# ZhiHuangHn/vtkCloudPoint

Hardware: AMD Instinct MI355X
Metric: Mpoints/s DBSCAN+label @10M pts (higher is better)
Workload: dtype f64; 1 GPU; C4: 10000000-pt cloud (half uniform background, 200 Gaussian blobs), one monolithic DBImproved.dbscan, metric L1_2D, eps 0.1, minPts 10; mode=single, points_total=10000000, points_per_gpu=10000000, clusters=27380, resident_in_hbm=True

## Files before the change

### include/vcp.h

```cpp
#ifndef VCP_H
#define VCP_H
#include <stdint.h>

#ifdef __cplusplus
extern "C" {
#endif

#define VCP_VERSION_MAJOR 0
#define VCP_VERSION_MINOR 1

typedef struct vcp_ctx vcp_ctx;

enum vcp_metric { VCP_L1_2D = 0, VCP_L2_2D = 1, VCP_L2_3D = 2, VCP_SIGNED_SUM_2D = 3 };

enum vcp_icp_stop { VCP_STOP_SSE_DELTA = 0, VCP_STOP_RMSE = 1 };

enum vcp_status {
  VCP_OK = 0,
  VCP_ERR_ARG = -1,
  VCP_ERR_EMPTY = -2,
  VCP_ERR_DEGENERATE = -3,
  VCP_ERR_INDEX = -4,
  VCP_ERR_TOO_LARGE = -5,
  VCP_ERR_NO_DEVICE = -6,
// ... 1 lines not shown
  VCP_ERR_UNSUPPORTED = -8,
  VCP_ERR_NOMEM = -9
};

int vcp_create(int device_id, vcp_ctx** out);
void vcp_destroy(vcp_ctx* ctx);
const char* vcp_last_error(const vcp_ctx* ctx);
int vcp_version(void);
int vcp_set_stream(vcp_ctx* ctx, void* hip_stream);
int vcp_dev_alloc(vcp_ctx* ctx, uint64_t bytes, void** dptr);
int vcp_dev_free(vcp_ctx* ctx, void* dptr);
int vcp_h2d(vcp_ctx* ctx, void* dst_dev, const void* src_host, uint64_t bytes);
int vcp_d2h(vcp_ctx* ctx, void* dst_host, const void* src_dev, uint64_t bytes);

int vcp_release_workspace(vcp_ctx* ctx);

int vcp_selftest_scan_dev(vcp_ctx* ctx, const uint32_t* d_in, uint32_t* d_out, int64_t n, int op, uint32_t* total);

int vcp_selftest_horn(const double sums[16], int64_t nd, double V[16], int use_v, double R1[9], double T1[3]);

int vcp_timing_enable(vcp_ctx* ctx, int on);
int vcp_timing_count(vcp_ctx* ctx);
int vcp_timing_get(vcp_ctx* ctx, int i, const char** name, float* ms);

int vcp_dbscan(vcp_ctx* ctx, const double* coords, int64_t n, int dim, int metric, double eps,
               int min_pts, int32_t cf_in, const uint8_t* in_mask, const uint8_t* in_classed,
               int32_t* labels, uint8_t* is_core, uint8_t* is_classed, int32_t* cf_out,
               int64_t* dist_evals);
int vcp_dbscan_dev(vcp_ctx* ctx, const double* d_coords, int64_t n, int dim, int metric, double eps,
                   int min_pts, int32_t cf_in, const uint8_t* d_in_classed, int32_t* d_labels,
// ... 166 lines not shown
```

### vtkcloudpoint_amd/_native.py

```python
import ctypes as C
import os

import numpy as np

_HERE = os.path.dirname(os.path.abspath(__file__))
LIB_PATH = os.path.join(_HERE, "libvcp.so")

L1_2D, L2_2D, L2_3D, SIGNED_SUM_2D = 0, 1, 2, 3
STOP_SSE_DELTA, STOP_RMSE = 0, 1

STATUS = {
    0: "VCP_OK", -1: "VCP_ERR_ARG", -2: "VCP_ERR_EMPTY", -3: "VCP_ERR_DEGENERATE", -4: "VCP_ERR_INDEX",
    -5: "VCP_ERR_TOO_LARGE", -6: "VCP_ERR_NO_DEVICE", -7: "VCP_ERR_HIP", -8: "VCP_ERR_UNSUPPORTED",
    -9: "VCP_ERR_NOMEM",
}

SYMBOLS = [
    "vcp_create", "vcp_destroy", "vcp_last_error", "vcp_version", "vcp_set_stream", "vcp_dev_alloc",
    "vcp_dev_free", "vcp_h2d", "vcp_d2h", "vcp_timing_enable", "vcp_timing_count", "vcp_timing_get",
    "vcp_dbscan", "vcp_dbscan_dev", "vcp_dbscan_blocks", "vcp_blocks_begin", "vcp_blocks_begin_dev",
    "vcp_blocks_share", "vcp_blocks_cluster_dev", "vcp_blocks_finish_dev", "vcp_centroids", "vcp_centroids_dev",
    "vcp_merge_centroids", "vcp_refresh_by_dictionary", "vcp_icp", "vcp_icp_dev", "vcp_icp_sums",
    "vcp_match", "vcp_mcc", "vcp_assign_truths", "vcp_icp_vtklike", "vcp_import_convert",
    "vcp_slab_begin", "vcp_slab_comps", "vcp_slab_finish", "vcp_release_workspace", "vcp_selftest_scan_dev",
    "vcp_centroids_weighted", "vcp_dbscan_blocks_keyed", "vcp_blocks_begin_keyed", "vcp_blocks_begin_keyed_dev",
    "vcp_selftest_horn", "vcp_create_multi", "vcp_destroy_multi", "vcp_multi_last_error", "vcp_multi_count",
    "vcp_multi_ctx", "vcp_dbscan_blocks_multi", "vcp_blocks_share_plan", "vcp_blocks_plan_dev", "vcp_blocks_plan_cuts",
    "vcp_blocks_build_dev", "vcp_blocks_finish_local_dev", "vcp_blocks_finish_zero_dev", "vcp_blocks_finish_zcoords_dev",
    "vcp_blocks_finish_pairs_dev", "vcp_scatter_pairs_dev", "vcp_kdist", "vcp_kdist_dev", "vcp_icp_multistart",
    "vcp_cluster_shapes", "vcp_cluster_shapes_dev", "vcp_cluster_filter", "vcp_cluster_filter_dev",
    "vcp_icp_sums_gated", "vcp_icp_gated", "vcp_match_unique", "vcp_match_unique_dev",
    "vcp_register_pairs", "vcp_register_pairs_dev", "vcp_selftest_register_pose",
]


class VcpError(RuntimeError):
    def __init__(self, code, msg):
        super().__init__("%s (%d): %s" % (STATUS.get(code, "?"), code, msg))
        self.code = code


_lib = None


def lib():
    global _lib
    if _lib is None:
        if not os.path.exists(LIB_PATH):
# ... 653 lines not shown
```

### vtkcloudpoint_amd/csrc/dbscan.hip

```cpp
#include <string.h>

#include <cmath>
#include <cstdlib>
#include <cstring>
#include <limits>
#include <vector>

#include "bounds.hpp"
#include "dbscan_engine.hpp"
#include "grid_common.hpp"

using namespace vcpg;

namespace {

#ifndef VCP_UNR2
#define VCP_UNR2 4
#endif
#ifndef VCP_UNR3
#define VCP_UNR3 2
#endif
#ifndef VCP_UNRW
#define VCP_UNRW 4
#endif
// ... 118 lines not shown
  uint32_t perblk;
  uint32_t nblk;
};

__device__ __forceinline__ uint32_t wl_fetch(const WorkList& w) {
  const uint32_t total = w.scan[w.nblk] - w.scan[0];
  const uint32_t x = blockIdx.x & 7u, i = blockIdx.x >> 3;
  const uint32_t c = (i / w.perblk) * 8u + x;
  const uint32_t lo = (uint32_t)(((uint64_t)total * c) / (8u * LCHUNK));
  const uint32_t hi = (uint32_t)(((uint64_t)total * (c + 1u)) / (8u * LCHUNK));
  const uint32_t t = lo + (i % w.perblk) * TPB + threadIdx.x;
  if (t >= hi) return NONE;
  return w.list[t];
}

__device__ __forceinline__ void wl_count(bool isE, bool isB, uint32_t blk, uint32_t* __restrict__ cntE,
                                         uint32_t* __restrict__ cntB) {
  __shared__ unsigned wc[2][TPB / 64];
  const unsigned long long mE = __ballot(isE), mB = __ballot(isB);
  if ((threadIdx.x & 63) == 0) {
    wc[0][threadIdx.x >> 6] = (unsigned)__popcll(mE);
    wc[1][threadIdx.x >> 6] = (unsigned)__popcll(mB);
  }
  __syncthreads();
  if (threadIdx.x == 0) {
    unsigned a = 0, b = 0;
    for (int k = 0; k < TPB / 64; k++) {
      a += wc[0][k];
      b += wc[1][k];
    }
// ... 46 lines not shown
  int NB;
  int core_cap;
};

__device__ __forceinline__ void wave_prefix_small(uint32_t v, uint32_t& pre, uint32_t& sum) {
  pre = 0;
  sum = 0;
#pragma unroll
  for (int b = 0; b < 4; b++) {
    const unsigned long long m = __ballot((v >> b) & 1u);
    pre += __builtin_amdgcn_mbcnt_hi((uint32_t)(m >> 32), __builtin_amdgcn_mbcnt_lo((uint32_t)m, 0u)) << b;
    sum += (uint32_t)__popcll(m) << b;
  }
}

__device__ __forceinline__ const uint32_t* nbr_list(const NbrOut& no, uint32_t p) {
  return no.nbr + (size_t)(p / TPB) * (size_t)(no.NB * TPB) + no.off[p];
}

__device__ __forceinline__ void nbr_flush(const NbrOut& no, const uint32_t* lnb, uint32_t* lout, int nrec, int64_t blk,
                                          int64_t p, bool live) {
  if (no.NB == 0) return;
  __shared__ uint32_t wtot[TPB / 64];
  const int lane = threadIdx.x & 63, w = threadIdx.x >> 6;
  uint32_t pre, wsum;
  wave_prefix_small((uint32_t)nrec, pre, wsum);
  if (lane == 0) wtot[w] = wsum;
  __syncthreads();
  uint32_t total = 0;
  for (int k = 0; k < TPB / 64; k++) {
    if (k < w) pre += wtot[k];
    total += wtot[k];
// ... 406 lines not shown
        const uint32_t jj = min(j0 + u, e - 1);
        cand[u] = (j0 + u < e) && (flags[jj] & F_EXPAND);
        if (GROUPED) cand[u] = cand[u] && sgroup[jj] == myg;
        load_pt32<GD>(sorted32, jj, rr[u]);
      }
#pragma unroll
      for (int u = 0; u < UNR; u++)
        if (first == me && cand[u] && within_scr<GD, METRIC>(qf, rr[u], sc, xs, me, j0 + u, thr)) first = j0 + u;
      if (first != me) return false;
    }
    return true;
  });
  if (first != me) parent[me] = first;
}

__global__ __launch_bounds__(TPB) void k_union_init_list(const uint8_t* __restrict__ flags, uint32_t* __restrict__ parent,
                                                        NbrOut no, WorkList wlE) {
  const uint32_t p = wl_fetch(wlE);
  if (p == NONE) return;
  const int nrec = flags[p] >> 4;
  const uint32_t* li = nbr_list(no, p);
  for (int k = 0; k < nrec; k++) {
    const uint32_t j = li[k];
    if (j < p && (flags[j] & F_EXPAND)) {
      parent[p] = j;
      return;
    }
  }
}

template <int JOIN>
__global__ __launch_bounds__(TPB) void k_flatten0(uint32_t* __restrict__ parent, WorkList wlE,
                                                 const uint8_t* __restrict__ flags, NbrOut no) {
  const uint32_t p = wl_fetch(wlE);
  if (p == NONE) return;
  uint32_t r = (uint32_t)p, x = ld_parent_cached(parent, r);
  if (x == r || JOIN == 2) {
    if (!JOIN) return;
    uint32_t rp = JOIN == 2 ? uf_root(parent, p) : p;
    const int nrec = flags[p] >> 4;
    const uint32_t* li = nbr_list(no, p);
    uint32_t s0 = NONE, s1 = NONE, s2 = NONE;
    for (int k = 0; k < nrec; k++) {
      const uint32_t j = li[k];
      if (!(flags[j] & F_EXPAND)) continue;
      const uint32_t y = ld_parent_cached(parent, j);
      if (y == rp || y == s0 || y == s1 || y == s2) continue;
      const uint32_t ry = uf_root(parent, y);
      const uint32_t rm = uf_root(parent, rp);
      s2 = s1;
      s1 = s0;
      s0 = rp;
      rp = (ry != rm) ? uf_link(parent, rm, ry) : rm;
      if (y != rp) s1 = y;
    }
    return;
  }
  while (x != r) {
    r = x;
    x = ld_parent_cached(parent, r);
  }
  __hip_atomic_store(&parent[p], r, __ATOMIC_RELAXED, __HIP_MEMORY_SCOPE_WAVEFRONT);
}

constexpr uint32_t CHUNK_MIXED = 0xFFFFFFFEu;
constexpr int DENSE_PER_CELL = 16;
__global__ __launch_bounds__(TPB) void k_chunkroot(const uint32_t* __restrict__ parent, CellTab ct,
                                                  uint32_t* __restrict__ chunkroot) {
  const uint32_t nin = *ct.nin;
  const int64_t p = (int64_t)blockIdx.x * TPB + threadIdx.x;
  const uint32_t x = p < nin ? parent[p] : NONE;
  const unsigned long long have = __ballot(x != NONE);
  uint32_t out = NONE;
  if (have) {
    const uint32_t r = (uint32_t)__shfl((int)x, __ffsll((long long)have) - 1, 64);
    out = __ballot(x != NONE && x != r) ? CHUNK_MIXED : r;
  }
// ... 90 lines not shown
        } else if (q1 == NONE) {
          q1 = x;
        } else {
          VCP_FLUSH();
          q0 = x;
        }
      }
    }
  }
  VCP_FLUSH();
  if (rp != me) __hip_atomic_store(&parent[me], rp, __ATOMIC_RELAXED, __HIP_MEMORY_SCOPE_AGENT);
}
#undef VCP_FLUSH
#undef VCP_JOIN

template <bool FILTER>
__global__ __launch_bounds__(TPB) void k_flatten(uint32_t* __restrict__ parent, const uint32_t* __restrict__ sord,
                                                uint32_t* __restrict__ minord, WorkList wlE) {
  const uint32_t p = wl_fetch(wlE);
  uint32_t r = NONE, v = NONE;
  if (p != NONE) {
    r = (uint32_t)p;
    uint32_t x = parent[r];
    while (x != r) {
      r = x;
      x = parent[r];
    }
    parent[p] = r;
    v = sord[p];
  }
  unsigned long long todo = __ballot(r != NONE);
  const int lane = threadIdx.x & 63;
  while (todo) {
    int leader = __ffsll((long long)todo) - 1;
    uint32_t lr = __shfl(r, leader, 64);
    bool mine = (r == lr);
    uint32_t m = mine ? v : NONE;
#pragma unroll
    for (int d = 32; d > 0; d >>= 1) m = min(m, (uint32_t)__shfl_xor((int)m, d, 64));
    if (lane == leader &&
        (!FILTER || m < __hip_atomic_load(&minord[lr], __ATOMIC_RELAXED, __HIP_MEMORY_SCOPE_AGENT)))
      atomicMin(&minord[lr], m);
    todo &= ~__ballot(mine);
  }
}

__device__ __forceinline__ uint32_t seed_rank(const uint32_t* __restrict__ bits, const uint32_t* __restrict__ pref,
                                              uint32_t m) {
  const uint32_t w = m >> 5;
  return pref[w] + (uint32_t)__popc(bits[w] & ((1u << (m & 31u)) - 1u));
}
__global__ __launch_bounds__(TPB) void k_seed_popc(const uint32_t* __restrict__ bits, uint32_t nw, uint32_t* __restrict__ cnt) {
  uint32_t w = blockIdx.x * TPB + threadIdx.x;
  if (w < nw) cnt[w] = (uint32_t)__popc(bits[w]);
}

__global__ __launch_bounds__(TPB) void k_seedflag(const uint32_t* __restrict__ parent, const uint32_t* __restrict__ minord,
                                                 uint32_t* __restrict__ seedflag, WorkList wlE) {
  const uint32_t p = wl_fetch(wlE);
  if (p == NONE) return;
  if (parent[p] == p) {
    const uint32_t m = minord[p];
    atomicOr(&seedflag[m >> 5], 1u << (m & 31u));
  }
}

__global__ __launch_bounds__(TPB) void k_rootk(const uint32_t* __restrict__ parent, const uint32_t* __restrict__ minord,
                                              const uint32_t* __restrict__ seedbits, const uint32_t* __restrict__ seedpref,
                                              uint32_t* __restrict__ rootk, uint32_t* __restrict__ clseed, WorkList wlE) {
  const uint32_t p = wl_fetch(wlE);
  if (p == NONE) return;
  if (parent[p] == p) {
    uint32_t k = seed_rank(seedbits, seedpref, minord[p]);
    rootk[p] = k;
    clseed[k] = minord[p];
  }
}

__device__ __forceinline__ void twice_add(unsigned twice, unsigned long long* __restrict__ counters) {
  __shared__ unsigned tw[TPB / 64];
  const unsigned long long m2 = __ballot(twice);
  if ((threadIdx.x & 63) == 0) tw[threadIdx.x >> 6] = (unsigned)__popcll(m2);
  __syncthreads();
  if (threadIdx.x == 0) {
    unsigned t = 0;
    for (int k = 0; k < TPB / 64; k++) t += tw[k];
    if (t) atomicAdd(&counters[CNT_TWICE + (blockIdx.x & (CNT_SPREAD - 1))], (unsigned long long)t);
  }
}

template <int GD, int METRIC, bool GROUPED>
__global__ __launch_bounds__(TPB) void k_border(ExactSrc xs, GridP g, double thr,
                                               CellTab ct,
                                               const int32_t* __restrict__ sgroup, const uint8_t* __restrict__ flags,
                                               const uint32_t* __restrict__ parent, const uint32_t* __restrict__ sord,
                                               const uint32_t* __restrict__ rootk, const uint32_t* __restrict__ clseed,
                                               uint32_t* __restrict__ labk, unsigned long long* __restrict__ counters,
// ... 31 lines not shown
          }
        }
        return true;
      });
      out = mx;
      if (mx != 0 && !(fl & F_CLASSED) && sord[p] - own_lo < own_span && sord[p] < clseed[mnk]) {
        twice = 1;
        if (GROUPED) atomicAdd(&group_twice[myg], 1u);
      }
    }
    labk[p] = (out << 2) | ((fl & F_CORE) ? 1u : 0u) | ((fl & F_CLASSED) ? 2u : 0u);
  }
  if (!GROUPED) twice_add(twice, counters);
}

template <bool GROUPED>
__global__ __launch_bounds__(TPB) void k_border_list(const int32_t* __restrict__ sgroup, const uint8_t* __restrict__ flags,
                                                    const uint32_t* __restrict__ sord, const uint32_t* __restrict__ rootk,
                                                    const uint32_t* __restrict__ clseed, uint32_t* __restrict__ labk,
                                                    unsigned long long* __restrict__ counters,
                                                    uint32_t* __restrict__ group_twice, NbrOut no, WorkList wlB) {
  const uint32_t p = wl_fetch(wlB);
  unsigned twice = 0;
  if (p != NONE) {
    const uint8_t fl = flags[p];
    const int nrec = fl >> 4;
    uint32_t mx = 0, mnk = NONE;
    const uint32_t* li = nbr_list(no, p);
    for (int k = 0; k < nrec; k++) {
      const uint32_t x = rootk[li[k]];
      if (x == NONE) continue;
      mx = max(mx, x + 1u);
      mnk = min(mnk, x);
    }
    if (mx != 0 && sord[p] < clseed[mnk]) twice = 1;
    labk[p] = (mx << 2) | ((fl & F_CORE) ? 1u : 0u) | ((fl & F_CLASSED) ? 2u : 0u);
  }
  if (GROUPED) {
    const int32_t g = twice ? sgroup[p] : -1;
    unsigned long long todo = __ballot(twice != 0);
    const int lane = threadIdx.x & 63;
    while (todo) {
      const int leader = __ffsll((long long)todo) - 1;
      const int32_t gl = __shfl(g, leader, 64);
      const unsigned long long same = __ballot(twice && g == gl);
      if (lane == leader) atomicAdd(&group_twice[gl], (uint32_t)__popcll(same));
      todo &= ~same;
    }
  } else {
    twice_add(twice, counters);
  }
}

__global__ __launch_bounds__(TPB) void k_labk_rest(const uint8_t* __restrict__ flags, const uint32_t* __restrict__ parent,
                                                  uint32_t* rootk, uint32_t* __restrict__ labk,
                                                  CellTab ct) {
  const uint32_t nin = *ct.nin;
  int64_t p = (int64_t)blockIdx.x * TPB + threadIdx.x;
  if (p >= nin) return;
  const uint8_t fl = flags[p];
  uint32_t k = NONE;
  if (fl & F_EXPAND) {
    const uint32_t r = parent[p];
    k = rootk[r];
    if (r != (uint32_t)p) rootk[p] = k;
// ... 244 lines not shown
  if (lo_ok && lo >= 0.0 && std::isfinite(lo)) {
    float l = (float)lo;
    if ((double)l > lo) l = std::nextafterf(l, -INFINITY);
    sc.lo = l;
  } else if (lo_ok && std::isinf(thr) && thr > 0) {
    sc.lo = 3.4028234663852886e38f;
  }
  return sc;
}

unsigned list_perblk(int64_t n) {
  const int64_t band = (n + 8 * LCHUNK - 1) / (8 * LCHUNK) + 1;
  return vcp_blocks(band, TPB);
}

struct Switches {
  int64_t cells_per_point;
  bool screen_off, lists_off, core_global;
  int core_cap, join_all;
};
const Switches& switches() {
  static const Switches sw = [] {
    Switches s;
    const char* e = getenv("VCP_CELL_BUDGET");
    const long v = e ? atol(e) : 32;
    s.cells_per_point = (int64_t)(v < 1 ? 1 : v > 4096 ? 4096 : v);
    s.screen_off = getenv("VCP_NO_SCREEN") != nullptr;
    s.lists_off = getenv("VCP_NO_LISTS") != nullptr;
    s.core_global = getenv("VCP_CORE_GLOBAL") != nullptr;
    s.core_cap = getenv("VCP_CORE_CAP") ? atoi(getenv("VCP_CORE_CAP")) : -1;
    s.join_all = getenv("VCP_JOIN_ALL") ? atoi(getenv("VCP_JOIN_ALL")) : -1;
    return s;
  }();
  return sw;
}

struct EnginePinned {
  double bounds[8];
  uint32_t unclassed;
  uint32_t n_comp;
  unsigned long long counters[CNT_WORDS];
};
static_assert(sizeof(EnginePinned) <= 1024, "the engine's region of vcp_ctx::pinned");
EnginePinned* engine_pinned(vcp_ctx* ctx) { return reinterpret_cast<EnginePinned*>(ctx->pinned); }

struct Call {
// ... 339 lines not shown
  }
  if (!tiled)
    VCP_LAUNCH(ctx, (k_core<GD, METRIC, GROUPED>), dim3(nb), dim3(TPB), 2 * lds_nb, st, c.xs, c.g, c.thr, c.min_pts, ws.ct,
                    ws.sgroup, ws.flags, ws.parent, ws.minord, ws.blkE, ws.blkB, no, ws.sorted32, c.sc, c.flags_set);
  VCP_TRY(vcp_exclusive_scan_u32(ctx, ws.blkE, ws.blkE, 2 * ((int64_t)nb + 2), nullptr));
  VCP_LAUNCH(ctx, k_wl_fill, dim3(nb), dim3(TPB), 0, st, ws.flags, ws.ct, ws.blkE, ws.blkB, ws.wlE.list, ws.wlB.list,
                  ws.seedflag, ws.nw, ws.counters, c.d_group_twice, (uint32_t)(GROUPED ? c.G : 0));
  return VCP_OK;
}

template <int GD, int METRIC, bool GROUPED>
int stage_union(vcp_ctx* ctx, const Call& c, const Workspace& ws, const Switches& sw) {
  hipStream_t st = ctx->stream;
  const int64_t n = c.n;
  const unsigned nb = c.nb, nbl = ws.nbl;
  const GridP& g = c.g;
  const NbrOut& no = c.no;
  vcp_phase(ctx, "union");
  const bool pre = GD == 2 || no.NB > 0;
  if (no.NB > 0) {
    VCP_LAUNCH(ctx, k_union_init_list, dim3(nbl), dim3(TPB), 0, st, ws.flags, ws.parent, no, ws.wlE);
    const bool all = sw.join_all >= 0 ? sw.join_all != 0 : (uint64_t)n >= (uint64_t)g.ncells;
    if (all) VCP_LAUNCH(ctx, k_flatten0<2>, dim3(nbl), dim3(TPB), 0, st, ws.parent, ws.wlE, ws.flags, no);
    else VCP_LAUNCH(ctx, k_flatten0<1>, dim3(nbl), dim3(TPB), 0, st, ws.parent, ws.wlE, ws.flags, no);
    VCP_LAUNCH(ctx, k_flatten0<0>, dim3(nbl), dim3(TPB), 0, st, ws.parent, ws.wlE, ws.flags, no);
  } else if (GD == 2) {
    VCP_LAUNCH(ctx, (k_union_init<GD, METRIC, GROUPED>), dim3(nbl), dim3(TPB), 0, st, c.xs, g, c.thr, ws.ct, ws.sgroup,
                    ws.flags, ws.parent, ws.wlE, ws.sorted32, c.sc);
    VCP_LAUNCH(ctx, k_flatten0<0>, dim3(nbl), dim3(TPB), 0, st, ws.parent, ws.wlE, ws.flags, no);
  }
  const bool dense = pre && (uint64_t)n > (uint64_t)DENSE_PER_CELL * g.ncells;
  if (dense) {
    VCP_TRY(vcp_ensure(ctx, ctx->b_aux0, ((size_t)nb * (TPB / 64) + 2) * 4));
    uint32_t* chunkroot = ctx->b_aux0.as<uint32_t>();
    VCP_LAUNCH(ctx, k_chunkroot, dim3(nb), dim3(TPB), 0, st, ws.parent, ws.ct, chunkroot);
    VCP_LAUNCH(ctx, (k_union<GD, METRIC, GROUPED, true, true>), dim3(nbl), dim3(TPB), 0, st, c.xs, g, c.thr, ws.ct,
                    ws.sgroup, ws.parent, ws.wlE, ws.sorted32, c.sc, chunkroot);
  } else if (pre)
    VCP_LAUNCH(ctx, (k_union<GD, METRIC, GROUPED, true>), dim3(nbl), dim3(TPB), 0, st, c.xs, g, c.thr, ws.ct, ws.sgroup,
                    ws.parent, ws.wlE, ws.sorted32, c.sc);
  else
    VCP_LAUNCH(ctx, (k_union<GD, METRIC, GROUPED, false>), dim3(nbl), dim3(TPB), 0, st, c.xs, g, c.thr, ws.ct, ws.sgroup,
                    ws.parent, ws.wlE, ws.sorted32, c.sc);
  return VCP_OK;
// ... 17 lines not shown
  ss.valid = true;
  ss.gd = c.gd;
  ss.metric = c.metric;
  ss.n = c.n;
  ss.n_comp = hn[0];
  ss.g = c.g;
  ss.thr = c.thr;
  ss.sc = c.sc;
  ss.xs = c.xs;
  ss.nb = nb;
  if (c.cf_out) *c.cf_out = (int32_t)hn[0];
  return VCP_OK;
}

template <bool GROUPED>
int stage_flatten_number(vcp_ctx* ctx, const Call& c, const Workspace& ws) {
  hipStream_t st = ctx->stream;
  const unsigned nbl = ws.nbl;
  vcp_phase(ctx, "flatten_number");
  if ((uint64_t)c.n >= (uint64_t)c.g.ncells)
    VCP_LAUNCH(ctx, k_flatten<true>, dim3(nbl), dim3(TPB), 0, st, ws.parent, ws.sord, ws.minord, ws.wlE);
  else
    VCP_LAUNCH(ctx, k_flatten<false>, dim3(nbl), dim3(TPB), 0, st, ws.parent, ws.sord, ws.minord, ws.wlE);
  if (!GROUPED && c.slab) return stage_slab_handoff(ctx, c, ws);
  VCP_LAUNCH(ctx, k_seedflag, dim3(nbl), dim3(TPB), 0, st, ws.parent, ws.minord, ws.seedflag, ws.wlE);
  VCP_LAUNCH(ctx, k_seed_popc, dim3(vcp_blocks(ws.nw, TPB)), dim3(TPB), 0, st, ws.seedflag, ws.nw, ws.seedpref);
  VCP_TRY(vcp_exclusive_scan_u32(ctx, ws.seedpref, ws.seedpref, ws.nw, ws.d_total));
  VCP_LAUNCH(ctx, k_rootk, dim3(nbl), dim3(TPB), 0, st, ws.parent, ws.minord, ws.seedflag, ws.seedpref, ws.rootk, ws.clseed,
                  ws.wlE);
  return VCP_OK;
}

template <int GD, int METRIC, bool GROUPED>
int stage_border(vcp_ctx* ctx, const Call& c, const Workspace& ws) {
  hipStream_t st = ctx->stream;
  vcp_phase(ctx, "border");
  VCP_LAUNCH(ctx, k_labk_rest, dim3(c.nb), dim3(TPB), 0, st, ws.flags, ws.parent, ws.rootk, ws.labk, ws.ct);
  if (c.no.NB > 0)
    VCP_LAUNCH(ctx, k_border_list<GROUPED>, dim3(ws.nbl), dim3(TPB), 0, st, ws.sgroup, ws.flags, ws.sord, ws.rootk,
                    ws.clseed, ws.labk, ws.counters, c.d_group_twice, c.no, ws.wlB);
  else
    VCP_LAUNCH(ctx, (k_border<GD, METRIC, GROUPED>), dim3(ws.nbl), dim3(TPB), 0, st, c.xs, c.g, c.thr, ws.ct, ws.sgroup,
                    ws.flags, ws.parent, ws.sord, ws.rootk, ws.clseed, ws.labk, ws.counters, c.d_group_twice, ws.wlB, 0u,
                    NONE, ws.sorted32, c.sc);
  return VCP_OK;
}

template <int GD, bool GROUPED>
int stage_output(vcp_ctx* ctx, const Call& c, const Workspace& ws) {
  hipStream_t st = ctx->stream;
  const int64_t n = c.n;
  const unsigned nb = c.nb;
  const DbscanExt* ext = c.ext;
  if (c.part_out) {
    GridOutputArgs oa;
    oa.n = n;
    oa.sord = ws.sord;
    oa.labk = ws.labk;
    oa.have_in_classed = c.d_in_classed != nullptr;
// ... 29 lines not shown
  c.thr = (METRIC == VCP_L1_2D) ? c.eps : l2_threshold(c.eps);
  if (!GROUPED && c.all_finite && !c.slab && box_measure<GD, METRIC>(c.h) <= c.thr) return run_all_pairs(ctx, c);

  double Emax = 0.0;
  VCP_TRY(grid_geometry(ctx, c, sw, Emax));
  c.sc = screen_bounds(METRIC, GD, METRIC == VCP_L1_2D ? c.thr * c.g.scale : c.thr * c.g.scale * c.g.scale, Emax * c.g.scale);
  if (sw.screen_off) c.sc = Screen{-1.0f, INFINITY};

  VCP_TRY(ws_reserve(ctx, c.n, c.nb, GD, GROUPED, c.g.ncells));
  const Workspace ws = ws_carve(ctx, c.n, c.nb, GROUPED, c.g.ncells);
  c.flags_set = c.d_in_classed != nullptr;
  c.part_out = !GROUPED && !c.d_ord && !c.slab && c.n <= ((int64_t)1 << 27);
  VCP_TRY(stage_grid_build(ctx, c, ws));
  VCP_TRY((stage_core<GD, METRIC, GROUPED>(ctx, c, ws, sw)));
  VCP_TRY((stage_union<GD, METRIC, GROUPED>(ctx, c, ws, sw)));
  VCP_TRY(stage_flatten_number<GROUPED>(ctx, c, ws));
  if (!GROUPED && c.slab) return VCP_OK;
  VCP_TRY((stage_border<GD, METRIC, GROUPED>(ctx, c, ws)));
  VCP_TRY((stage_output<GD, GROUPED>(ctx, c, ws)));

  Totals t;
  VCP_TRY(read_totals(ctx, ws, t));
  const unsigned long long unclassed = c.d_in_classed ? t.unclassed : (unsigned long long)c.n;
  if (c.cf_out) *c.cf_out = c.cf_in + (int32_t)t.K;
  if (c.dist_evals)
    *c.dist_evals = GROUPED ? (int64_t)t.group_evals : (int64_t)(unclassed + t.twice + t.K - t.slot0) * c.n;
  return VCP_OK;
}

template <int GD, int METRIC>
int run_slab_finish(vcp_ctx* ctx, const SlabState& ss, const uint32_t* d_map_rep, const uint32_t* d_map_k,
                    const int32_t* d_tab_gid, uint32_t own_lo, uint32_t own_span, int32_t* d_labels,
                    uint8_t* d_is_classed, int64_t* twice) {
// ... 85 lines not shown
  Call c{d_coords, n, stride, metric, eps, min_pts, cf_in, d_in_classed, d_labels, d_is_core, d_is_classed, cf_out,
         dist_evals, ext};
  call_derive(c);
  if (!(eps >= 0.0)) {
    if (grouped) return vcp_fail(ctx, VCP_ERR_ARG, "grouped DBSCAN needs eps >= 0");
    return run_degenerate(ctx, c);
  }
  if (grouped) return run_dbscan<2, VCP_L1_2D, true>(ctx, c);
  if (metric == VCP_L1_2D) return run_dbscan<2, VCP_L1_2D, false>(ctx, c);
  if (metric == VCP_L2_2D) return run_dbscan<2, VCP_L2_2D, false>(ctx, c);
  return run_dbscan<3, VCP_L2_3D, false>(ctx, c);
}

extern "C" {

void vcp_slab_state_free(vcp_ctx* ctx) {
  delete ctx->slab;
  ctx->slab = nullptr;
}

int vcp_slab_begin(vcp_ctx* ctx, const double* d_coords, int64_t n, int dim, int metric, double eps, int min_pts,
                   const uint8_t* d_noexpand, const uint32_t* d_ord, uint32_t* d_rep, uint8_t* d_is_core,
                   int64_t* n_comp) {
  if (!ctx) return VCP_ERR_ARG;
  if (n <= 0) return vcp_fail(ctx, VCP_ERR_ARG, "vcp_slab_begin needs n > 0");
  if (!d_ord || !d_rep || !n_comp) return vcp_fail(ctx, VCP_ERR_ARG, "null buffer");
  if (!(eps >= 0.0) || std::isinf(eps)) return vcp_fail(ctx, VCP_ERR_ARG, "staged DBSCAN needs a finite eps >= 0");
  DbscanExt ext;
  ext.d_ord = d_ord;
  ext.slab = true;
// ... 126 lines not shown
```

Baseline: 7019 Mpoints/s.

## Process multiple worklist entries per thread with batched neighbor-list loads

```diff
diff --git a/include/vcp.h b/include/vcp.h
--- a/include/vcp.h
+++ b/include/vcp.h
@@ -39,6 +39,8 @@
 int vcp_d2h(vcp_ctx* ctx, void* dst_host, const void* src_dev, uint64_t bytes);
 
 int vcp_release_workspace(vcp_ctx* ctx);
+
+int vcp_worklist_entries(void);
 
 int vcp_selftest_scan_dev(vcp_ctx* ctx, const uint32_t* d_in, uint32_t* d_out, int64_t n, int op, uint32_t* total);
 
diff --git a/vtkcloudpoint_amd/_native.py b/vtkcloudpoint_amd/_native.py
--- a/vtkcloudpoint_amd/_native.py
+++ b/vtkcloudpoint_amd/_native.py
@@ -30,8 +30,12 @@
     "vcp_blocks_finish_pairs_dev", "vcp_scatter_pairs_dev", "vcp_kdist", "vcp_kdist_dev", "vcp_icp_multistart",
     "vcp_cluster_shapes", "vcp_cluster_shapes_dev", "vcp_cluster_filter", "vcp_cluster_filter_dev",
     "vcp_icp_sums_gated", "vcp_icp_gated", "vcp_match_unique", "vcp_match_unique_dev",
-    "vcp_register_pairs", "vcp_register_pairs_dev", "vcp_selftest_register_pose",
+    "vcp_register_pairs", "vcp_register_pairs_dev", "vcp_selftest_register_pose", "vcp_worklist_entries",
 ]
+
+
+def worklist_entries():
+    return int(lib().vcp_worklist_entries())
 
 
 class VcpError(RuntimeError):
diff --git a/vtkcloudpoint_amd/csrc/dbscan.hip b/vtkcloudpoint_amd/csrc/dbscan.hip
--- a/vtkcloudpoint_amd/csrc/dbscan.hip
+++ b/vtkcloudpoint_amd/csrc/dbscan.hip
@@ -4,6 +4,7 @@
 #include <cstdlib>
 #include <cstring>
 #include <limits>
+#include <type_traits>
 #include <vector>
 
 #include "bounds.hpp"
@@ -156,6 +157,35 @@
   return w.list[t];
 }
 
+constexpr int WL_EMAX = 4;
+__host__ __device__ constexpr uint32_t wl_perblk(uint32_t perblk, int E) {
+  return (perblk + (uint32_t)E - 1u) / (uint32_t)E;
+}
+template <int E>
+__device__ __forceinline__ void wl_fetch_n(const WorkList& w, uint32_t (&p)[E]) {
+  static_assert(E >= 1 && E <= WL_EMAX, "entries per thread");
+  const uint32_t total = w.scan[w.nblk] - w.scan[0];
+  const uint32_t per = wl_perblk(w.perblk, E);
+  const uint32_t x = blockIdx.x & 7u, i = blockIdx.x >> 3;
+  const uint32_t c = (i / per) * 8u + x;
+  const uint32_t lo = (uint32_t)(((uint64_t)total * c) / (8u * LCHUNK));
+  const uint32_t hi = (uint32_t)(((uint64_t)total * (c + 1u)) / (8u * LCHUNK));
+  const uint32_t t0 = lo + (i % per) * (uint32_t)(E * TPB) + threadIdx.x;
+#pragma unroll
+  for (int e = 0; e < E; e++) {
+    const uint32_t t = t0 + (uint32_t)(e * TPB);
+    const uint32_t v = w.list[t < hi ? t : 0u];
+    p[e] = t < hi ? v : NONE;
+  }
+}
+__device__ __forceinline__ uint32_t wl_safe(uint32_t p) { return p != NONE ? p : 0u; }
+__device__ __forceinline__ void loaded_here(uint32_t v) { asm volatile("" ::"v"(v)); }
+constexpr int LBATCH = 4;
+__device__ __forceinline__ uint32_t list_word(const uint32_t* li, int nrec, int k, const uint32_t* idle) {
+  const uint32_t* src = nrec > 0 ? li + min(k, nrec - 1) : idle;
+  return *src;
+}
+
 __device__ __forceinline__ void wl_count(bool isE, bool isB, uint32_t blk, uint32_t* __restrict__ cntE,
                                          uint32_t* __restrict__ cntB) {
   __shared__ unsigned wc[2][TPB / 64];
@@ -232,8 +262,8 @@
   }
 }
 
-__device__ __forceinline__ const uint32_t* nbr_list(const NbrOut& no, uint32_t p) {
-  return no.nbr + (size_t)(p / TPB) * (size_t)(no.NB * TPB) + no.off[p];
+__device__ __forceinline__ const uint32_t* nbr_list(const NbrOut& no, uint32_t p, uint32_t of) {
+  return no.nbr + (size_t)(p / TPB) * (size_t)(no.NB * TPB) + of;
 }
 
 __device__ __forceinline__ void nbr_flush(const NbrOut& no, const uint32_t* lnb, uint32_t* lout, int nrec, int64_t blk,
@@ -670,53 +700,137 @@
   if (first != me) parent[me] = first;
 }
 
+template <int E>
 __global__ __launch_bounds__(TPB) void k_union_init_list(const uint8_t* __restrict__ flags, uint32_t* __restrict__ parent,
                                                         NbrOut no, WorkList wlE) {
-  const uint32_t p = wl_fetch(wlE);
-  if (p == NONE) return;
-  const int nrec = flags[p] >> 4;
-  const uint32_t* li = nbr_list(no, p);
-  for (int k = 0; k < nrec; k++) {
-    const uint32_t j = li[k];
-    if (j < p && (flags[j] & F_EXPAND)) {
-      parent[p] = j;
-      return;
-    }
-  }
-}
-
-template <int JOIN>
-__global__ __launch_bounds__(TPB) void k_flatten0(uint32_t* __restrict__ parent, WorkList wlE,
-                                                 const uint8_t* __restrict__ flags, NbrOut no) {
-  const uint32_t p = wl_fetch(wlE);
-  if (p == NONE) return;
-  uint32_t r = (uint32_t)p, x = ld_parent_cached(parent, r);
-  if (x == r || JOIN == 2) {
-    if (!JOIN) return;
-    uint32_t rp = JOIN == 2 ? uf_root(parent, p) : p;
-    const int nrec = flags[p] >> 4;
-    const uint32_t* li = nbr_list(no, p);
-    uint32_t s0 = NONE, s1 = NONE, s2 = NONE;
-    for (int k = 0; k < nrec; k++) {
-      const uint32_t j = li[k];
-      if (!(flags[j] & F_EXPAND)) continue;
-      const uint32_t y = ld_parent_cached(parent, j);
-      if (y == rp || y == s0 || y == s1 || y == s2) continue;
-      const uint32_t ry = uf_root(parent, y);
+  constexpr int LB = E * LBATCH > 8 ? 8 / E : LBATCH;
+  uint32_t p[E];
+  wl_fetch_n<E>(wlE, p);
+  uint8_t fl[E];
+  uint32_t of[E];
+#pragma unroll
+  for (int e = 0; e < E; e++) {
+    fl[e] = flags[wl_safe(p[e])];
+    of[e] = no.off[wl_safe(p[e])];
+  }
+#pragma unroll
+  for (int e = 0; e < E; e++) loaded_here(of[e]);
+  int nrec[E];
+  const uint32_t* li[E];
+  uint32_t first[E];
+#pragma unroll
+  for (int e = 0; e < E; e++) {
+    nrec[e] = p[e] != NONE ? fl[e] >> 4 : 0;
+    li[e] = nbr_list(no, wl_safe(p[e]), of[e]);
+    first[e] = NONE;
+  }
+  for (int k0 = 0;; k0 += LB) {
+    bool more = false;
+#pragma unroll
+    for (int e = 0; e < E; e++) more = more || (first[e] == NONE && k0 < nrec[e]);
+    if (!more) break;
+    uint32_t j[E][LB];
+    uint8_t fj[E][LB];
+#pragma unroll
+    for (int e = 0; e < E; e++)
+#pragma unroll
+      for (int u = 0; u < LB; u++) j[e][u] = list_word(li[e], nrec[e], k0 + u, wlE.list);
+#pragma unroll
+    for (int e = 0; e < E; e++)
+#pragma unroll
+      for (int u = 0; u < LB; u++) {
+        const bool ok = k0 + u < nrec[e] && j[e][u] < p[e];
+        fj[e][u] = flags[ok ? j[e][u] : wl_safe(p[e])];
+        if (!ok) fj[e][u] = 0;
+      }
+#pragma unroll
+    for (int e = 0; e < E; e++)
+#pragma unroll
+      for (int u = 0; u < LB; u++)
+        if (first[e] == NONE && (fj[e][u] & F_EXPAND)) first[e] = j[e][u];
+  }
+#pragma unroll
+  for (int e = 0; e < E; e++)
+    if (first[e] != NONE) parent[p[e]] = first[e];
+}
+
+__device__ __forceinline__ void join_along_list(uint32_t* __restrict__ parent, const uint8_t* __restrict__ flags,
+                                                const NbrOut& no, uint32_t p, uint32_t rp) {
+  const uint8_t fl = flags[p];
+  const uint32_t of = no.off[p];
+  loaded_here(of);
+  const int nrec = fl >> 4;
+  const uint32_t* li = nbr_list(no, p, of);
+  uint32_t s0 = NONE, s1 = NONE, s2 = NONE;
+  for (int k0 = 0; k0 < nrec; k0 += LBATCH) {
+    uint32_t j[LBATCH], y[LBATCH];
+    uint8_t fj[LBATCH];
+#pragma unroll
+    for (int u = 0; u < LBATCH; u++) j[u] = li[min(k0 + u, nrec - 1)];
+#pragma unroll
+    for (int u = 0; u < LBATCH; u++) {
+      fj[u] = flags[j[u]];
+      y[u] = ld_parent_cached(parent, j[u]);
+      if (k0 + u >= nrec) fj[u] = 0;
+    }
+#pragma unroll
+    for (int u = 0; u < LBATCH; u++) {
+      if (!(fj[u] & F_EXPAND)) continue;
+      if (y[u] == rp || y[u] == s0 || y[u] == s1 || y[u] == s2) continue;
+      const uint32_t ry = uf_root(parent, y[u]);
       const uint32_t rm = uf_root(parent, rp);
       s2 = s1;
       s1 = s0;
       s0 = rp;
       rp = (ry != rm) ? uf_link(parent, rm, ry) : rm;
-      if (y != rp) s1 = y;
-    }
-    return;
-  }
-  while (x != r) {
-    r = x;
-    x = ld_parent_cached(parent, r);
-  }
-  __hip_atomic_store(&parent[p], r, __ATOMIC_RELAXED, __HIP_MEMORY_SCOPE_WAVEFRONT);
+      if (y[u] != rp) s1 = y[u];
+    }
+  }
+}
+
+template <int JOIN, int E>
+__global__ __launch_bounds__(TPB) void k_flatten0(uint32_t* __restrict__ parent, WorkList wlE,
+                                                 const uint8_t* __restrict__ flags, NbrOut no) {
+  uint32_t p[E];
+  wl_fetch_n<E>(wlE, p);
+  bool root[E];
+  if (JOIN != 2) {
+    uint32_t r[E], x[E];
+#pragma unroll
+    for (int e = 0; e < E; e++) {
+      r[e] = wl_safe(p[e]);
+      x[e] = ld_parent_cached(parent, r[e]);
+    }
+#pragma unroll
+    for (int e = 0; e < E; e++) {
+      if (p[e] == NONE) x[e] = r[e];
+      root[e] = p[e] != NONE && x[e] == r[e];
+    }
+    for (;;) {
+      bool any = false;
+#pragma unroll
+      for (int e = 0; e < E; e++) {
+        any = any || x[e] != r[e];
+        r[e] = x[e];
+      }
+      if (!any) break;
+#pragma unroll
+      for (int e = 0; e < E; e++) {
+        x[e] = ld_parent_cached(parent, r[e]);
+        if (p[e] == NONE) x[e] = r[e];
+      }
+    }
+#pragma unroll
+    for (int e = 0; e < E; e++)
+      if (p[e] != NONE && !root[e]) __hip_atomic_store(&parent[p[e]], r[e], __ATOMIC_RELAXED, __HIP_MEMORY_SCOPE_WAVEFRONT);
+  }
+  if (JOIN) {
+#pragma unroll
+    for (int e = 0; e < E; e++) {
+      if (JOIN == 2 ? p[e] != NONE : root[e])
+        join_along_list(parent, flags, no, p[e], JOIN == 2 ? uf_root(parent, p[e]) : p[e]);
+    }
+  }
 }
 
 constexpr uint32_t CHUNK_MIXED = 0xFFFFFFFEu;
@@ -837,34 +951,59 @@
 #undef VCP_FLUSH
 #undef VCP_JOIN
 
-template <bool FILTER>
+template <bool FILTER, int E>
 __global__ __launch_bounds__(TPB) void k_flatten(uint32_t* __restrict__ parent, const uint32_t* __restrict__ sord,
                                                 uint32_t* __restrict__ minord, WorkList wlE) {
-  const uint32_t p = wl_fetch(wlE);
-  uint32_t r = NONE, v = NONE;
-  if (p != NONE) {
-    r = (uint32_t)p;
-    uint32_t x = parent[r];
-    while (x != r) {
-      r = x;
-      x = parent[r];
-    }
-    parent[p] = r;
-    v = sord[p];
-  }
-  unsigned long long todo = __ballot(r != NONE);
+  uint32_t p[E];
+  wl_fetch_n<E>(wlE, p);
+  uint32_t r[E], x[E], v[E];
+#pragma unroll
+  for (int e = 0; e < E; e++) {
+    r[e] = wl_safe(p[e]);
+    x[e] = parent[r[e]];
+    v[e] = sord[r[e]];
+  }
+#pragma unroll
+  for (int e = 0; e < E; e++)
+    if (p[e] == NONE) x[e] = r[e];
+  for (;;) {
+    bool any = false;
+#pragma unroll
+    for (int e = 0; e < E; e++) {
+      any = any || x[e] != r[e];
+      r[e] = x[e];
+    }
+    if (!any) break;
+#pragma unroll
+    for (int e = 0; e < E; e++) {
+      x[e] = parent[r[e]];
+      if (p[e] == NONE) x[e] = r[e];
+    }
+  }
+#pragma unroll
+  for (int e = 0; e < E; e++) {
+    if (p[e] != NONE) {
+      parent[p[e]] = r[e];
+    } else {
+      r[e] = v[e] = NONE;
+    }
+  }
   const int lane = threadIdx.x & 63;
-  while (todo) {
-    int leader = __ffsll((long long)todo) - 1;
-    uint32_t lr = __shfl(r, leader, 64);
-    bool mine = (r == lr);
-    uint32_t m = mine ? v : NONE;
-#pragma unroll
-    for (int d = 32; d > 0; d >>= 1) m = min(m, (uint32_t)__shfl_xor((int)m, d, 64));
-    if (lane == leader &&
-        (!FILTER || m < __hip_atomic_load(&minord[lr], __ATOMIC_RELAXED, __HIP_MEMORY_SCOPE_AGENT)))
-      atomicMin(&minord[lr], m);
-    todo &= ~__ballot(mine);
+#pragma unroll
+  for (int e = 0; e < E; e++) {
+    unsigned long long todo = __ballot(r[e] != NONE);
+    while (todo) {
+      int leader = __ffsll((long long)todo) - 1;
+      uint32_t lr = __shfl(r[e], leader, 64);
+      bool mine = (r[e] == lr);
+      uint32_t m = mine ? v[e] : NONE;
+#pragma unroll
+      for (int d = 32; d > 0; d >>= 1) m = min(m, (uint32_t)__shfl_xor((int)m, d, 64));
+      if (lane == leader &&
+          (!FILTER || m < __hip_atomic_load(&minord[lr], __ATOMIC_RELAXED, __HIP_MEMORY_SCOPE_AGENT)))
+        atomicMin(&minord[lr], m);
+      todo &= ~__ballot(mine);
+    }
   }
 }
 
@@ -878,32 +1017,71 @@
   if (w < nw) cnt[w] = (uint32_t)__popc(bits[w]);
 }
 
+template <int E>
 __global__ __launch_bounds__(TPB) void k_seedflag(const uint32_t* __restrict__ parent, const uint32_t* __restrict__ minord,
                                                  uint32_t* __restrict__ seedflag, WorkList wlE) {
-  const uint32_t p = wl_fetch(wlE);
-  if (p == NONE) return;
-  if (parent[p] == p) {
-    const uint32_t m = minord[p];
-    atomicOr(&seedflag[m >> 5], 1u << (m & 31u));
-  }
-}
-
+  uint32_t p[E];
+  wl_fetch_n<E>(wlE, p);
+  uint32_t x[E], m[E];
+#pragma unroll
+  for (int e = 0; e < E; e++) {
+    x[e] = parent[wl_safe(p[e])];
+    m[e] = minord[wl_safe(p[e])];
+  }
+#pragma unroll
+  for (int e = 0; e < E; e++)
+    if (p[e] != NONE && x[e] == p[e]) atomicOr(&seedflag[m[e] >> 5], 1u << (m[e] & 31u));
+}
+
+template <int E>
 __global__ __launch_bounds__(TPB) void k_rootk(const uint32_t* __restrict__ parent, const uint32_t* __restrict__ minord,
                                               const uint32_t* __restrict__ seedbits, const uint32_t* __restrict__ seedpref,
                                               uint32_t* __restrict__ rootk, uint32_t* __restrict__ clseed, WorkList wlE) {
-  const uint32_t p = wl_fetch(wlE);
-  if (p == NONE) return;
-  if (parent[p] == p) {
-    uint32_t k = seed_rank(seedbits, seedpref, minord[p]);
-    rootk[p] = k;
-    clseed[k] = minord[p];
-  }
+  uint32_t p[E];
+  wl_fetch_n<E>(wlE, p);
+  uint32_t x[E], m[E], pw[E], bw[E];
+#pragma unroll
+  for (int e = 0; e < E; e++) {
+    x[e] = parent[wl_safe(p[e])];
+    m[e] = minord[wl_safe(p[e])];
+  }
+#pragma unroll
+  for (int e = 0; e < E; e++) {
+    pw[e] = bw[e] = 0u;
+    if (p[e] != NONE && x[e] == p[e]) {
+      pw[e] = seedpref[m[e] >> 5];
+      bw[e] = seedbits[m[e] >> 5];
+    }
+  }
+#pragma unroll
+  for (int e = 0; e < E; e++)
+    if (p[e] != NONE && x[e] == p[e]) {
+      const uint32_t k = pw[e] + (uint32_t)__popc(bw[e] & ((1u << (m[e] & 31u)) - 1u));
+      rootk[p[e]] = k;
+      clseed[k] = m[e];
+    }
 }
 
 __device__ __forceinline__ void twice_add(unsigned twice, unsigned long long* __restrict__ counters) {
   __shared__ unsigned tw[TPB / 64];
   const unsigned long long m2 = __ballot(twice);
   if ((threadIdx.x & 63) == 0) tw[threadIdx.x >> 6] = (unsigned)__popcll(m2);
+  __syncthreads();
+  if (threadIdx.x == 0) {
+    unsigned t = 0;
+    for (int k = 0; k < TPB / 64; k++) t += tw[k];
+    if (t) atomicAdd(&counters[CNT_TWICE + (blockIdx.x & (CNT_SPREAD - 1))], (unsigned long long)t);
+  }
+}
+
+template <int E>
+__device__ __forceinline__ void twice_add_n(unsigned c, unsigned long long* __restrict__ counters) {
+  static_assert(E <= 7, "three bits");
+  __shared__ unsigned tw[TPB / 64];
+  unsigned ws = 0;
+#pragma unroll
+  for (int b = 0; b < (E > 3 ? 3 : E > 1 ? 2 : 1); b++) ws += (unsigned)__popcll(__ballot((c >> b) & 1u)) << b;
+  if ((threadIdx.x & 63) == 0) tw[threadIdx.x >> 6] = ws;
   __syncthreads();
   if (threadIdx.x == 0) {
     unsigned t = 0;
@@ -965,41 +1143,92 @@
   if (!GROUPED) twice_add(twice, counters);
 }
 
-template <bool GROUPED>
+template <bool GROUPED, int E>
 __global__ __launch_bounds__(TPB) void k_border_list(const int32_t* __restrict__ sgroup, const uint8_t* __restrict__ flags,
                                                     const uint32_t* __restrict__ sord, const uint32_t* __restrict__ rootk,
                                                     const uint32_t* __restrict__ clseed, uint32_t* __restrict__ labk,
                                                     unsigned long long* __restrict__ counters,
                                                     uint32_t* __restrict__ group_twice, NbrOut no, WorkList wlB) {
-  const uint32_t p = wl_fetch(wlB);
-  unsigned twice = 0;
-  if (p != NONE) {
-    const uint8_t fl = flags[p];
-    const int nrec = fl >> 4;
-    uint32_t mx = 0, mnk = NONE;
-    const uint32_t* li = nbr_list(no, p);
-    for (int k = 0; k < nrec; k++) {
-      const uint32_t x = rootk[li[k]];
-      if (x == NONE) continue;
-      mx = max(mx, x + 1u);
-      mnk = min(mnk, x);
-    }
-    if (mx != 0 && sord[p] < clseed[mnk]) twice = 1;
-    labk[p] = (mx << 2) | ((fl & F_CORE) ? 1u : 0u) | ((fl & F_CLASSED) ? 2u : 0u);
+  constexpr int LB = E * LBATCH > 8 ? 8 / E : LBATCH;
+  uint32_t p[E];
+  wl_fetch_n<E>(wlB, p);
+  uint8_t fl[E];
+  uint32_t of[E], so[E];
+#pragma unroll
+  for (int e = 0; e < E; e++) {
+    fl[e] = flags[wl_safe(p[e])];
+    of[e] = no.off[wl_safe(p[e])];
+    so[e] = sord[wl_safe(p[e])];
+  }
+#pragma unroll
+  for (int e = 0; e < E; e++) loaded_here(of[e]);
+  int nrec[E], nmax = 0;
+  const uint32_t* li[E];
+  uint32_t mx[E], mnk[E];
+#pragma unroll
+  for (int e = 0; e < E; e++) {
+    nrec[e] = p[e] != NONE ? fl[e] >> 4 : 0;
+    nmax = max(nmax, nrec[e]);
+    li[e] = nbr_list(no, wl_safe(p[e]), of[e]);
+    mx[e] = 0;
+    mnk[e] = NONE;
+  }
+  for (int k0 = 0; k0 < nmax; k0 += LB) {
+    uint32_t j[E][LB], x[E][LB];
+#pragma unroll
+    for (int e = 0; e < E; e++)
+#pragma unroll
+      for (int u = 0; u < LB; u++) j[e][u] = list_word(li[e], nrec[e], k0 + u, wlB.list);
+#pragma unroll
+    for (int e = 0; e < E; e++)
+#pragma unroll
+      for (int u = 0; u < LB; u++) {
+        x[e][u] = rootk[k0 + u < nrec[e] ? j[e][u] : wl_safe(p[e])];
+        if (k0 + u >= nrec[e]) x[e][u] = NONE;
+      }
+#pragma unroll
+    for (int e = 0; e < E; e++)
+#pragma unroll
+      for (int u = 0; u < LB; u++) {
+        if (x[e][u] == NONE) continue;
+        mx[e] = max(mx[e], x[e][u] + 1u);
+        mnk[e] = min(mnk[e], x[e][u]);
+      }
+  }
+  uint32_t cs[E];
+#pragma unroll
+  for (int e = 0; e < E; e++) {
+    cs[e] = clseed[mx[e] != 0 ? mnk[e] : 0u];
+  }
+  bool twice[E];
+  unsigned ntwice = 0;
+#pragma unroll
+  for (int e = 0; e < E; e++) {
+    twice[e] = mx[e] != 0 && so[e] < cs[e];
+    ntwice += twice[e] ? 1u : 0u;
+    if (p[e] != NONE) labk[p[e]] = (mx[e] << 2) | ((fl[e] & F_CORE) ? 1u : 0u) | ((fl[e] & F_CLASSED) ? 2u : 0u);
   }
   if (GROUPED) {
-    const int32_t g = twice ? sgroup[p] : -1;
-    unsigned long long todo = __ballot(twice != 0);
+    int32_t g[E];
+#pragma unroll
+    for (int e = 0; e < E; e++) {
+      g[e] = -1;
+      if (twice[e]) g[e] = sgroup[p[e]];
+    }
     const int lane = threadIdx.x & 63;
-    while (todo) {
-      const int leader = __ffsll((long long)todo) - 1;
-      const int32_t gl = __shfl(g, leader, 64);
-      const unsigned long long same = __ballot(twice && g == gl);
-      if (lane == leader) atomicAdd(&group_twice[gl], (uint32_t)__popcll(same));
-      todo &= ~same;
+#pragma unroll
+    for (int e = 0; e < E; e++) {
+      unsigned long long todo = __ballot(twice[e]);
+      while (todo) {
+        const int leader = __ffsll((long long)todo) - 1;
+        const int32_t gl = __shfl(g[e], leader, 64);
+        const unsigned long long same = __ballot(twice[e] && g[e] == gl);
+        if (lane == leader) atomicAdd(&group_twice[gl], (uint32_t)__popcll(same));
+        todo &= ~same;
+      }
     }
   } else {
-    twice_add(twice, counters);
+    twice_add_n<E>(ntwice, counters);
   }
 }
 
@@ -1274,10 +1503,24 @@
   return vcp_blocks(band, TPB);
 }
 
+constexpr int WL_E_UNION_INIT = 4, WL_E_FLATTEN0 = 4, WL_E_FLATTEN0_JOIN = 2, WL_E_FLATTEN = 4, WL_E_SEEDFLAG = 4,
+              WL_E_ROOTK = 4, WL_E_BORDER = 2;
+template <class F>
+int wl_with_e(int own, int sw_e, uint32_t perblk, F&& f) {
+  const int e = sw_e ? sw_e : own;
+  const dim3 gl(8u * LCHUNK * wl_perblk(perblk, e));
+  switch (e) {
+    case 1: return f(std::integral_constant<int, 1>{}, gl);
+    case 2: return f(std::integral_constant<int, 2>{}, gl);
+    default: return f(std::integral_constant<int, WL_EMAX>{}, gl);
+  }
+}
+
 struct Switches {
   int64_t cells_per_point;
   bool screen_off, lists_off, core_global;
   int core_cap, join_all;
+  int wl_e;
 };
 const Switches& switches() {
   static const Switches sw = [] {
@@ -1290,6 +1533,8 @@
     s.core_global = getenv("VCP_CORE_GLOBAL") != nullptr;
     s.core_cap = getenv("VCP_CORE_CAP") ? atoi(getenv("VCP_CORE_CAP")) : -1;
     s.join_all = getenv("VCP_JOIN_ALL") ? atoi(getenv("VCP_JOIN_ALL")) : -1;
+    const int we = getenv("VCP_WL_E") ? atoi(getenv("VCP_WL_E")) : 0;
+    s.wl_e = (we == 1 || we == 2 || we == 4) ? we : 0;
     return s;
   }();
   return sw;
@@ -1659,20 +1904,40 @@
   hipStream_t st = ctx->stream;
   const int64_t n = c.n;
   const unsigned nb = c.nb, nbl = ws.nbl;
+  const uint32_t pb = ws.wlE.perblk;
   const GridP& g = c.g;
   const NbrOut& no = c.no;
   vcp_phase(ctx, "union");
   const bool pre = GD == 2 || no.NB > 0;
   if (no.NB > 0) {
-    VCP_LAUNCH(ctx, k_union_init_list, dim3(nbl), dim3(TPB), 0, st, ws.flags, ws.parent, no, ws.wlE);
+    VCP_TRY(wl_with_e(WL_E_UNION_INIT, sw.wl_e, pb, [&](auto E, dim3 gl) -> int {
+      constexpr int e = decltype(E)::value;
+      VCP_LAUNCH(ctx, k_union_init_list<e>, gl, dim3(TPB), 0, st, ws.flags, ws.parent, no, ws.wlE);
+      return VCP_OK;
+    }));
     const bool all = sw.join_all >= 0 ? sw.join_all != 0 : (uint64_t)n >= (uint64_t)g.ncells;
-    if (all) VCP_LAUNCH(ctx, k_flatten0<2>, dim3(nbl), dim3(TPB), 0, st, ws.parent, ws.wlE, ws.flags, no);
-    else VCP_LAUNCH(ctx, k_flatten0<1>, dim3(nbl), dim3(TPB), 0, st, ws.parent, ws.wlE, ws.flags, no);
-    VCP_LAUNCH(ctx, k_flatten0<0>, dim3(nbl), dim3(TPB), 0, st, ws.parent, ws.wlE, ws.flags, no);
+    VCP_TRY(wl_with_e(WL_E_FLATTEN0_JOIN, sw.wl_e, pb, [&](auto E, dim3 gl) -> int {
+      constexpr int e = decltype(E)::value;
+      if (all) {
+        VCP_LAUNCH(ctx, (k_flatten0<2, e>), gl, dim3(TPB), 0, st, ws.parent, ws.wlE, ws.flags, no);
+      } else {
+        VCP_LAUNCH(ctx, (k_flatten0<1, e>), gl, dim3(TPB), 0, st, ws.parent, ws.wlE, ws.flags, no);
+      }
+      return VCP_OK;
+    }));
+    VCP_TRY(wl_with_e(WL_E_FLATTEN0, sw.wl_e, pb, [&](auto E, dim3 gl) -> int {
+      constexpr int e = decltype(E)::value;
+      VCP_LAUNCH(ctx, (k_flatten0<0, e>), gl, dim3(TPB), 0, st, ws.parent, ws.wlE, ws.flags, no);
+      return VCP_OK;
+    }));
   } else if (GD == 2) {
     VCP_LAUNCH(ctx, (k_union_init<GD, METRIC, GROUPED>), dim3(nbl), dim3(TPB), 0, st, c.xs, g, c.thr, ws.ct, ws.sgroup,
                     ws.flags, ws.parent, ws.wlE, ws.sorted32, c.sc);
-    VCP_LAUNCH(ctx, k_flatten0<0>, dim3(nbl), dim3(TPB), 0, st, ws.parent, ws.wlE, ws.flags, no);
+    VCP_TRY(wl_with_e(WL_E_FLATTEN0, sw.wl_e, pb, [&](auto E, dim3 gl) -> int {
+      constexpr int e = decltype(E)::value;
+      VCP_LAUNCH(ctx, (k_flatten0<0, e>), gl, dim3(TPB), 0, st, ws.parent, ws.wlE, ws.flags, no);
+      return VCP_OK;
+    }));
   }
   const bool dense = pre && (uint64_t)n > (uint64_t)DENSE_PER_CELL * g.ncells;
   if (dense) {
@@ -1720,35 +1985,53 @@
 }
 
 template <bool GROUPED>
-int stage_flatten_number(vcp_ctx* ctx, const Call& c, const Workspace& ws) {
+int stage_flatten_number(vcp_ctx* ctx, const Call& c, const Workspace& ws, const Switches& sw) {
   hipStream_t st = ctx->stream;
-  const unsigned nbl = ws.nbl;
+  const uint32_t pb = ws.wlE.perblk;
   vcp_phase(ctx, "flatten_number");
-  if ((uint64_t)c.n >= (uint64_t)c.g.ncells)
-    VCP_LAUNCH(ctx, k_flatten<true>, dim3(nbl), dim3(TPB), 0, st, ws.parent, ws.sord, ws.minord, ws.wlE);
-  else
-    VCP_LAUNCH(ctx, k_flatten<false>, dim3(nbl), dim3(TPB), 0, st, ws.parent, ws.sord, ws.minord, ws.wlE);
+  VCP_TRY(wl_with_e(WL_E_FLATTEN, sw.wl_e, pb, [&](auto E, dim3 gl) -> int {
+    constexpr int e = decltype(E)::value;
+    if ((uint64_t)c.n >= (uint64_t)c.g.ncells) {
+      VCP_LAUNCH(ctx, (k_flatten<true, e>), gl, dim3(TPB), 0, st, ws.parent, ws.sord, ws.minord, ws.wlE);
+    } else {
+      VCP_LAUNCH(ctx, (k_flatten<false, e>), gl, dim3(TPB), 0, st, ws.parent, ws.sord, ws.minord, ws.wlE);
+    }
+    return VCP_OK;
+  }));
   if (!GROUPED && c.slab) return stage_slab_handoff(ctx, c, ws);
-  VCP_LAUNCH(ctx, k_seedflag, dim3(nbl), dim3(TPB), 0, st, ws.parent, ws.minord, ws.seedflag, ws.wlE);
+  VCP_TRY(wl_with_e(WL_E_SEEDFLAG, sw.wl_e, pb, [&](auto E, dim3 gl) -> int {
+    constexpr int e = decltype(E)::value;
+    VCP_LAUNCH(ctx, k_seedflag<e>, gl, dim3(TPB), 0, st, ws.parent, ws.minord, ws.seedflag, ws.wlE);
+    return VCP_OK;
+  }));
   VCP_LAUNCH(ctx, k_seed_popc, dim3(vcp_blocks(ws.nw, TPB)), dim3(TPB), 0, st, ws.seedflag, ws.nw, ws.seedpref);
   VCP_TRY(vcp_exclusive_scan_u32(ctx, ws.seedpref, ws.seedpref, ws.nw, ws.d_total));
-  VCP_LAUNCH(ctx, k_rootk, dim3(nbl), dim3(TPB), 0, st, ws.parent, ws.minord, ws.seedflag, ws.seedpref, ws.rootk, ws.clseed,
-                  ws.wlE);
+  VCP_TRY(wl_with_e(WL_E_ROOTK, sw.wl_e, pb, [&](auto E, dim3 gl) -> int {
+    constexpr int e = decltype(E)::value;
+    VCP_LAUNCH(ctx, k_rootk<e>, gl, dim3(TPB), 0, st, ws.parent, ws.minord, ws.seedflag, ws.seedpref, ws.rootk, ws.clseed,
+                    ws.wlE);
+    return VCP_OK;
+  }));
   return VCP_OK;
 }
 
 template <int GD, int METRIC, bool GROUPED>
-int stage_border(vcp_ctx* ctx, const Call& c, const Workspace& ws) {
+int stage_border(vcp_ctx* ctx, const Call& c, const Workspace& ws, const Switches& sw) {
   hipStream_t st = ctx->stream;
   vcp_phase(ctx, "border");
   VCP_LAUNCH(ctx, k_labk_rest, dim3(c.nb), dim3(TPB), 0, st, ws.flags, ws.parent, ws.rootk, ws.labk, ws.ct);
-  if (c.no.NB > 0)
-    VCP_LAUNCH(ctx, k_border_list<GROUPED>, dim3(ws.nbl), dim3(TPB), 0, st, ws.sgroup, ws.flags, ws.sord, ws.rootk,
-                    ws.clseed, ws.labk, ws.counters, c.d_group_twice, c.no, ws.wlB);
-  else
+  if (c.no.NB > 0) {
+    VCP_TRY(wl_with_e(WL_E_BORDER, sw.wl_e, ws.wlB.perblk, [&](auto E, dim3 gl) -> int {
+      constexpr int e = decltype(E)::value;
+      VCP_LAUNCH(ctx, (k_border_list<GROUPED, e>), gl, dim3(TPB), 0, st, ws.sgroup, ws.flags, ws.sord, ws.rootk, ws.clseed,
+                      ws.labk, ws.counters, c.d_group_twice, c.no, ws.wlB);
+      return VCP_OK;
+    }));
+  } else {
     VCP_LAUNCH(ctx, (k_border<GD, METRIC, GROUPED>), dim3(ws.nbl), dim3(TPB), 0, st, c.xs, c.g, c.thr, ws.ct, ws.sgroup,
                     ws.flags, ws.parent, ws.sord, ws.rootk, ws.clseed, ws.labk, ws.counters, c.d_group_twice, ws.wlB, 0u,
                     NONE, ws.sorted32, c.sc);
+  }
   return VCP_OK;
 }
 
@@ -1808,9 +2091,9 @@
   VCP_TRY(stage_grid_build(ctx, c, ws));
   VCP_TRY((stage_core<GD, METRIC, GROUPED>(ctx, c, ws, sw)));
   VCP_TRY((stage_union<GD, METRIC, GROUPED>(ctx, c, ws, sw)));
-  VCP_TRY(stage_flatten_number<GROUPED>(ctx, c, ws));
+  VCP_TRY(stage_flatten_number<GROUPED>(ctx, c, ws, sw));
   if (!GROUPED && c.slab) return VCP_OK;
-  VCP_TRY((stage_border<GD, METRIC, GROUPED>(ctx, c, ws)));
+  VCP_TRY((stage_border<GD, METRIC, GROUPED>(ctx, c, ws, sw)));
   VCP_TRY((stage_output<GD, GROUPED>(ctx, c, ws)));
 
   Totals t;
@@ -1926,6 +2209,8 @@
 
 extern "C" {
 
+int vcp_worklist_entries(void) { return WL_EMAX; }
+
 void vcp_slab_state_free(vcp_ctx* ctx) {
   delete ctx->slab;
   ctx->slab = nullptr;
```

After: 6674 Mpoints/s. -4.9%, worse.
